# sparisi/pvr_habitat

Measured on AMD Instinct MI355X. Metric: frames/sec embedded (ResNet50, 256x256), higher is better.
Workload: dtype f16; 1 GPU; configs[1]: ResNet50 (MoCo-v2 layout) frozen, 256x256 uint8 frames resident in HBM, batch 256/GPU, random-init synthetic weights, f16 storage / MFMA inputs with fp32 accumulation (the product default, inside the 1e-3 parity bound; configs[1] names bf16); global_batch=256, frame=256, chunk=256, batches_in_flight=2, parallelism=frame shards, no collective (dp1)

## Files before the change

### include/pvr_hip.h

```cpp
#ifndef PVR_HIP_H
#define PVR_HIP_H

#include <stddef.h>
#include <stdint.h>

#ifdef __cplusplus
extern "C" {
#endif

typedef int pvr_status;
#define PVR_OK 0
#define PVR_ERR_INVALID 1
#define PVR_ERR_MISSING_WEIGHT 2
#define PVR_ERR_HIP 3
#define PVR_ERR_STATE 4

#define PVR_BF16 0
#define PVR_F16 1
#define PVR_F32 2
#define PVR_F32S 3

#define PVR_ARCH_RESNET50 0
#define PVR_ARCH_RESNET50_L4 1
#define PVR_ARCH_RESNET50_L3 2
// ... 69 lines not shown
                         const void *residual_dev, void *out_dev, int32_t n, int32_t h, int32_t w,
                         int32_t cin, int32_t cout, int32_t kh, int32_t kw, int32_t stride, int32_t pad,
                         int32_t relu, int32_t out_f32, int32_t dtype, void *hip_stream);
pvr_status pvr_op_conv2d_splitk(const void *in_dev, const void *wgt_dev, const float *bias_dev, const void *residual_dev, void *out_dev, float *scratch_dev,
                                int32_t ksplit, int32_t n, int32_t h, int32_t w, int32_t cin, int32_t cout, int32_t kh, int32_t kw, int32_t stride,
                                int32_t pad, int32_t relu, int32_t out_f32, int32_t dtype, void *hip_stream);
pvr_status pvr_op_bneck_frame(const void *t1_dev, const void *w2_dev, const float *b2_dev, const void *w3_dev, const float *b3_dev,
                              const void *residual_dev, void *y_dev, void *t2_out_dev, const void *w1n_dev, const float *b1n_dev, void *t1n_dev,
                              const void *w1f_dev, const float *b1f_dev, int32_t n, int32_t phases, int32_t dtype, void *hip_stream);
pvr_status pvr_op_pack_frag_weights(const void *w_dev, void *out_dev, int32_t rows, int32_t k, void *hip_stream);
pvr_status pvr_debug_bneck_frame_stamps(const void *t1_dev, const void *w2_dev, const float *b2_dev, const void *w3_dev, const float *b3_dev,
                                        const void *residual_dev, void *y_dev, const void *w1n_dev, const float *b1n_dev, void *t1n_dev,
                                        const void *w1f_dev, const float *b1f_dev, int32_t n, int32_t dtype, uint64_t *stamps_dev, void *hip_stream);
int64_t pvr_debug_bneck_frame_launches(void);
pvr_status pvr_op_conv_wfrag(const void *in_dev, const void *wgt_packed_dev, const float *bias_dev, const void *residual_dev, void *out_dev, int32_t n,
                             int32_t h, int32_t w, int32_t cin, int32_t cout, int32_t kh, int32_t kw, int32_t stride, int32_t pad, int32_t relu,
                             int32_t out_f32, int32_t dtype, void *hip_stream);
pvr_status pvr_op_conv2d_dual(const void *in_dev, const void *in2_dev, const void *wgt_dev, const float *bias_dev, void *out_dev, int32_t n, int32_t h,
                              int32_t w, int32_t cin, int32_t cout, int32_t kh, int32_t kw, int32_t stride, int32_t pad, int32_t h2, int32_t w2,
                              int32_t cin2, int32_t stride2, int32_t relu, int32_t dtype, void *hip_stream);
pvr_status pvr_op_conv_wfrag_pool(const void *in_dev, const void *wgt_packed_dev, const float *bias_dev, const void *residual_dev, float *pool_out_dev,
                                  int64_t pool_stride, int32_t n, int32_t cin, int32_t cout, int32_t dtype, void *hip_stream);
int64_t pvr_debug_conv_wfrag_launches(void);
pvr_status pvr_op_split16_pack_weights(const float *w_dev, void *out_dev, int32_t rows, int32_t k, void *hip_stream);
pvr_status pvr_op_conv2d_split16(const float *in_dev, const void *wgt_split_dev, const float *bias_dev, const float *residual_dev, float *out_dev, int32_t n,
                                 int32_t h, int32_t w, int32_t cin, int32_t cout, int32_t k, int32_t stride, int32_t pad, int32_t relu, void *hip_stream);
pvr_status pvr_op_conv2d_f32(const float *in_dev, const float *wgt_dev, const float *bias_dev, const float *residual_dev, float *out_dev, int32_t n,
                             int32_t h, int32_t w, int32_t cin, int32_t cout, int32_t k, int32_t stride, int32_t pad, int32_t relu, void *hip_stream);
int64_t pvr_debug_conv_split16_launches(void);
pvr_status pvr_op_stem_split16(const float *img_padded_dev, const void *wgt_split_dev, const float *bias_dev, float *out_dev, int32_t n, int32_t S,
                               void *hip_stream);
int64_t pvr_debug_stem_split16_launches(void);
pvr_status pvr_debug_set_conv_algo(int32_t algo);
pvr_status pvr_file_sizes(const char *const *paths, int32_t n, int64_t *sizes, int32_t threads);
pvr_status pvr_read_files(const char *const *paths, int32_t n, uint8_t *dst, const int64_t *offsets, int32_t threads);
pvr_status pvr_stage_copy(void *dst, const void *src, int64_t rows, int64_t row_bytes, int64_t src_row_stride, int64_t run_bytes,
                          int64_t run_stride, int32_t threads);
int64_t pvr_png_scratch_bytes(int32_t n, int32_t h, int32_t w);
pvr_status pvr_png_decode(const uint8_t *files_dev, const int64_t *offsets_dev, int32_t n, int32_t h, int32_t w, uint8_t *out_dev,
                          uint8_t *scratch_dev, int64_t scratch_bytes, int32_t *status_dev, void *hip_stream);

int64_t pvr_debug_conv_expand_launches(void);
int64_t pvr_debug_pp_persistent_launches(void);
pvr_status pvr_op_avgpool(const void *in_dev, float *out_dev, int64_t out_stride, int32_t n, int32_t hw,
                          int32_t c, int32_t in_f32, int32_t dtype, void *hip_stream);
pvr_status pvr_op_avgpool2(const void *in_dev, void *out_dev, int32_t n, int32_t h, int32_t w, int32_t c, int32_t dtype, void *hip_stream);
// ... 21 lines not shown
```

### pvr_habitat_amd/_lib.py

```python
import ctypes as C
import os

_HERE = os.path.dirname(os.path.abspath(__file__))
LIB_PATH = os.environ.get('PVR_LIB') or os.path.join(_HERE, 'lib', 'libpvr_hip.so')

PVR_BF16, PVR_F16, PVR_F32, PVR_F32S = 0, 1, 2, 3
ARCH_RESNET50, ARCH_RESNET50_L4, ARCH_RESNET50_L3 = 0, 1, 2


class EncoderDesc(C.Structure):
    _fields_ = [('arch', C.c_int32), ('dtype', C.c_int32), ('max_batch', C.c_int32), ('chunk', C.c_int32),
                ('resize', C.c_int32), ('crop', C.c_int32), ('mean', C.c_float * 3), ('std_', C.c_float * 3)]


_lib = None

_SIGS = {
    'pvr_version': (C.c_char_p, []),
    'pvr_has_experiments': (C.c_int32, []),
    'pvr_debug_stem_u8_geometry_ok': (C.c_int32, [C.c_void_p, C.c_int32, C.c_int32, C.c_int32, C.c_int32]),
    'pvr_encoder_set_host_backend': (C.c_int, [C.c_void_p, C.c_int32]),
    'pvr_stage_copy': (C.c_int, [C.c_void_p, C.c_void_p, C.c_int64, C.c_int64, C.c_int64, C.c_int64, C.c_int64, C.c_int32]),
    'pvr_last_error': (C.c_size_t, [C.c_char_p, C.c_size_t]),
    'pvr_encoder_create': (C.c_int, [C.POINTER(EncoderDesc), C.POINTER(C.c_void_p)]),
# ... 19 lines not shown
    'pvr_encoder_profile': (C.c_int, [C.c_void_p, C.c_void_p, C.c_int32, C.c_int32, C.c_int32, C.c_void_p, C.c_int64, C.c_void_p,
                                      C.c_void_p, C.c_void_p, C.c_int32, C.POINTER(C.c_int32)]),
    'pvr_encoder_profile_span': (C.c_int, [C.c_void_p, C.c_void_p, C.c_int32, C.c_int32, C.c_int32, C.c_void_p, C.c_int64, C.c_void_p, C.c_int32, C.c_int32,
                                           C.POINTER(C.c_float)]),
    'pvr_op_preprocess': (C.c_int, [C.c_void_p, C.c_int32, C.c_int32, C.c_int32, C.c_int32, C.c_int32, C.c_void_p, C.c_int32, C.c_void_p]),
    'pvr_op_stem': (C.c_int, [C.c_void_p, C.c_void_p, C.c_void_p, C.c_void_p, C.c_int32, C.c_int32, C.c_void_p]),
    'pvr_op_stem_pool': (C.c_int, [C.c_void_p] * 4 + [C.c_int32] * 2 + [C.c_void_p] * 3 + [C.c_int32, C.c_void_p]),
    'pvr_op_stem_pool_u8': (C.c_int, [C.c_void_p] + [C.c_int32] * 5 + [C.c_void_p] * 3 + [C.c_int32] + [C.c_void_p] * 3 + [C.c_int32, C.c_void_p]),
    'pvr_debug_stem_c1_pack': (C.c_int, [C.c_void_p, C.c_void_p]),
    'pvr_op_conv2d_splitk': (C.c_int, [C.c_void_p] * 6 + [C.c_int32] * 13 + [C.c_void_p]),
    'pvr_op_avgpool2': (C.c_int, [C.c_void_p, C.c_void_p] + [C.c_int32] * 5 + [C.c_void_p]),
    'pvr_op_attnpool_tokens': (C.c_int, [C.c_void_p] * 3 + [C.c_int32] * 4 + [C.c_void_p]),
    'pvr_op_nhwc_to_chw': (C.c_int, [C.c_void_p, C.c_void_p, C.c_int64] + [C.c_int32] * 4 + [C.c_void_p]),
    'pvr_op_f32_to_h': (C.c_int, [C.c_void_p, C.c_void_p, C.c_int64, C.c_int32, C.c_void_p]),
    'pvr_op_h_to_f32': (C.c_int, [C.c_void_p, C.c_void_p, C.c_int64, C.c_int32, C.c_void_p]),
    'pvr_op_maxpool': (C.c_int, [C.c_void_p, C.c_void_p, C.c_int32, C.c_int32, C.c_int32, C.c_int32, C.c_int32, C.c_void_p]),
    'pvr_op_conv2d': (C.c_int, [C.c_void_p, C.c_void_p, C.c_void_p, C.c_void_p, C.c_void_p] + [C.c_int32] * 12 + [C.c_void_p]),
    'pvr_op_avgpool': (C.c_int, [C.c_void_p, C.c_void_p, C.c_int64, C.c_int32, C.c_int32, C.c_int32, C.c_int32, C.c_int32, C.c_void_p]),
    'pvr_debug_convert': (C.c_int, [C.c_void_p, C.c_void_p, C.c_int64, C.c_int32]),
    'pvr_op_bneck_frame': (C.c_int, [C.c_void_p] * 13 + [C.c_int32] * 3 + [C.c_void_p]),
    'pvr_debug_bneck_frame_launches': (C.c_int64, []),
    'pvr_op_conv_wfrag': (C.c_int, [C.c_void_p] * 5 + [C.c_int32] * 12 + [C.c_void_p]),
    'pvr_debug_conv_wfrag_launches': (C.c_int64, []),
    'pvr_op_conv_wfrag_pool': (C.c_int, [C.c_void_p] * 5 + [C.c_int64] + [C.c_int32] * 4 + [C.c_void_p]),
    'pvr_op_conv2d_dual': (C.c_int, [C.c_void_p] * 5 + [C.c_int32] * 15 + [C.c_void_p]),
    'pvr_op_pack_frag_weights': (C.c_int, [C.c_void_p, C.c_void_p, C.c_int32, C.c_int32, C.c_void_p]),
    'pvr_debug_bneck_frame_stamps': (C.c_int, [C.c_void_p] * 12 + [C.c_int32] * 2 + [C.c_void_p] * 2),
    'pvr_encoder_check_range': (C.c_int, [C.c_void_p, C.c_void_p, C.c_int32, C.c_int32, C.c_int32, C.c_void_p, C.c_int64, C.c_void_p, C.POINTER(C.c_int32)]),
    'pvr_encoder_debug_set_switch': (C.c_int, [C.c_void_p, C.c_char_p, C.c_int32]),
    'pvr_encoder_launch_kernel': (C.c_int32, [C.c_void_p, C.c_int32, C.c_int32, C.c_char_p, C.c_int32]),
    'pvr_op_split16_pack_weights': (C.c_int, [C.c_void_p, C.c_void_p, C.c_int32, C.c_int32, C.c_void_p]),
    'pvr_op_conv2d_split16': (C.c_int, [C.c_void_p] * 5 + [C.c_int32] * 9 + [C.c_void_p]),
    'pvr_op_conv2d_f32': (C.c_int, [C.c_void_p] * 5 + [C.c_int32] * 9 + [C.c_void_p]),
    'pvr_debug_conv_split16_launches': (C.c_int64, []),
    'pvr_op_stem_split16': (C.c_int, [C.c_void_p] * 4 + [C.c_int32] * 2 + [C.c_void_p]),
    'pvr_debug_stem_split16_launches': (C.c_int64, []),
    'pvr_op_attention': (C.c_int, [C.c_void_p, C.c_void_p, C.c_int32, C.c_int32, C.c_int32, C.c_int32, C.c_int32, C.c_void_p]),
    'pvr_op_layernorm': (C.c_int, [C.c_void_p] * 8 + [C.c_int32] * 3 + [C.c_float, C.c_int32, C.c_int32, C.c_void_p]),
    'pvr_op_cls_head': (C.c_int, [C.c_void_p] * 5 + [C.c_int64] + [C.c_int32] * 4 + [C.c_float, C.c_void_p]),
    'pvr_op_nonfinite_flag': (C.c_int, [C.c_void_p, C.c_int64, C.c_int64, C.c_int64, C.c_void_p, C.c_void_p]),
    'pvr_trainer_create': (C.c_int, [C.POINTER(EncoderDesc), C.POINTER(C.c_void_p)]),
    'pvr_trainer_destroy': (None, [C.c_void_p]),
    'pvr_trainer_out_size': (C.c_int32, [C.c_void_p]),
    'pvr_trainer_param_count': (C.c_int64, [C.c_void_p]),
    'pvr_trainer_workspace_bytes': (C.c_int64, [C.c_void_p]),
    'pvr_trainer_param_name': (C.c_int32, [C.c_void_p, C.c_int32, C.c_char_p, C.c_int32]),
# ... 62 lines not shown
```

### pvr_habitat_amd/csrc/api.hip

```cpp
#include <stdarg.h>
#include "encoder_internal.h"
#include "sample_rng.h"
#include <dlfcn.h>

namespace pvr {

static thread_local std::string g_err;

void set_error(const char *fmt, ...) {
    char buf[1024];
    va_list ap;
    va_start(ap, fmt);
    vsnprintf(buf, sizeof buf, fmt, ap);
    va_end(ap);
    g_err = buf;
}
const std::string &last_error() { return g_err; }

namespace {
typedef int (*roctx_push_fn)(const char *);
typedef int (*roctx_pop_fn)();
struct Roctx {
    roctx_push_fn push = nullptr;
    roctx_pop_fn pop = nullptr;
    Roctx() {
        const char *e = getenv("PVR_ROCTX");
        if (!e || atoi(e) == 0) return;
        for (const char *name : {"librocprofiler-sdk-roctx.so", "librocprofiler-sdk-roctx.so.1", "libroctx64.so", "libroctx64.so.4"}) {
            if (void *h = dlopen(name, RTLD_NOW | RTLD_GLOBAL)) {
                push = (roctx_push_fn)dlsym(h, "roctxRangePushA");
                pop = (roctx_pop_fn)dlsym(h, "roctxRangePop");
                if (push && pop) return;
                push = nullptr; pop = nullptr;
            }
        }
    }
};
const Roctx &roctx() { static Roctx r; return r; }
}
void trace_push(const char *name) { if (roctx().push) roctx().push(name); }
void trace_pop() { if (roctx().pop) roctx().pop(); }

long long conv_expand_launches();
long long bneck_frame_launches();
long long pp_persistent_launches();
long long conv_wfrag_launches();
long long conv_split16_launches();
pvr_status launch_split16_pack(const float *w, void *out, int rows, int K, hipStream_t stream);
pvr_status launch_conv_split16(const float *in, const void *wsp, const float *bias, const float *res, float *out, int n, int h, int w, int cin,
                               int cout, int k, int stride, int pad, int relu, hipStream_t stream, float *out2 = nullptr, int n1 = 0, void *out16 = nullptr,
                               int terms = 3);

static void *g_zero = nullptr;
static pvr_status zero_page(void **out) {
    if (!g_zero) {
        PVR_HIP_TRY(hipMalloc(&g_zero, PVR_ZERO_BYTES));
        PVR_HIP_TRY(hipMemset(g_zero, 0, PVR_ZERO_BYTES));
        PVR_HIP_TRY(hipDeviceSynchronize());
    }
    *out = g_zero;
    return PVR_OK;
}

}

using namespace pvr;

extern "C" {

// ... 18 lines not shown
    return launch_bneck_frame(op_switches(), t1, w2, b2, w3, b3, residual, y, nullptr, n, (w1n ? 7 : 3) | (w1f ? 8 : 0), dtype, (hipStream_t)stream, (unsigned long long *)stamps_dev,
                              w1n, b1n, t1n, w1f, b1f);
}
pvr_status pvr_op_conv_wfrag(const void *in, const void *wgt_packed, const float *bias, const void *residual, void *out, int32_t n, int32_t h, int32_t w,
                             int32_t cin, int32_t cout, int32_t kh, int32_t kw, int32_t stride, int32_t pad, int32_t relu, int32_t out_f32, int32_t dtype,
                             void *stream) {
    PVR_REQUIRE(n > 0 && h > 0 && w > 0, "pvr_op_conv_wfrag: empty input");
    return launch_conv_wfrag(op_switches(), in, wgt_packed, bias, residual, out, n, h, w, cin, cout, kh, kw, stride, pad, relu, out_f32, dtype, (hipStream_t)stream);
}
pvr_status pvr_op_conv2d_dual(const void *in, const void *in2, const void *wgt, const float *bias, void *out, int32_t n, int32_t h, int32_t w, int32_t cin,
                              int32_t cout, int32_t kh, int32_t kw, int32_t stride, int32_t pad, int32_t h2, int32_t w2, int32_t cin2, int32_t stride2,
                              int32_t relu, int32_t dtype, void *stream) {
    PVR_REQUIRE(in && in2 && wgt && bias && out && n > 0, "pvr_op_conv2d_dual: null argument");
    PVR_REQUIRE(dtype == PVR_BF16 || dtype == PVR_F16, "pvr_op_conv2d_dual: 16-bit storage types only");
    return launch_conv_pp256(op_switches(), in, wgt, bias, nullptr, out, n, h, w, cin, cout, kh, kw, stride, pad, relu, 0, 0, dtype, 224, (hipStream_t)stream, in2, h2, w2,
                             cin2, stride2);
}
pvr_status pvr_op_conv_wfrag_pool(const void *in, const void *wgt_packed, const float *bias, const void *residual, float *pool_out, int64_t pool_stride,
                                  int32_t n, int32_t cin, int32_t cout, int32_t dtype, void *stream) {
    PVR_REQUIRE(n > 0 && pool_out, "pvr_op_conv_wfrag_pool: empty input");
    return launch_conv_wfrag(op_switches(), in, wgt_packed, bias, residual, nullptr, n, 7, 7, cin, cout, 1, 1, 1, 0, 1, 1, dtype, (hipStream_t)stream, pool_out, pool_stride);
}
int64_t pvr_debug_conv_wfrag_launches(void) { return (int64_t)conv_wfrag_launches(); }
pvr_status pvr_op_split16_pack_weights(const float *w, void *out, int32_t rows, int32_t k, void *stream) {
    return launch_split16_pack(w, out, rows, k, (hipStream_t)stream);
}
pvr_status pvr_op_conv2d_split16(const float *in, const void *wgt_split, const float *bias, const float *residual, float *out, int32_t n, int32_t h,
                                 int32_t w, int32_t cin, int32_t cout, int32_t k, int32_t stride, int32_t pad, int32_t relu, void *stream) {
    PVR_REQUIRE(n > 0 && h > 0 && w > 0, "pvr_op_conv2d_split16: empty input");
    return launch_conv_split16(in, wgt_split, bias, residual, out, n, h, w, cin, cout, k, stride, pad, relu, (hipStream_t)stream);
}
pvr_status pvr_op_conv2d_f32(const float *in, const float *wgt, const float *bias, const float *residual, float *out, int32_t n, int32_t h, int32_t w,
                             int32_t cin, int32_t cout, int32_t k, int32_t stride, int32_t pad, int32_t relu, void *stream) {
    PVR_REQUIRE(in && wgt && bias && out && n > 0, "pvr_op_conv2d_f32: null argument");
    return launch_conv_f32(in, wgt, bias, residual, out, n, h, w, cin, cout, k, stride, pad, relu, (hipStream_t)stream);
}
int64_t pvr_debug_conv_split16_launches(void) { return (int64_t)conv_split16_launches(); }
pvr_status pvr_op_stem_split16(const float *img_padded, const void *wgt_split, const float *bias, float *out, int32_t n, int32_t S, void *stream) {
    return launch_stem_split16(img_padded, wgt_split, bias, out, n, S, (hipStream_t)stream);
}
int64_t pvr_debug_stem_split16_launches(void) { return (int64_t)stem_split16_launches(); }
int64_t pvr_debug_pp_persistent_launches(void) { return (int64_t)pp_persistent_launches(); }

size_t pvr_last_error(char *buf, size_t cap) {
    const std::string &e = last_error();
    if (buf && cap) {
// ... 168 lines not shown
```

### pvr_habitat_amd/csrc/conv_wfrag.hip

```cpp
#include "encoder_internal.h"

namespace pvr {

struct WFP {
    const u16 *in, *w, *res;
    const float *bias;
    void *out;
    int M, H, W, Cin, Cout, Ho, Wo, KH, KW, stride, pad, act;
    int MT, NCT;
    int nch, cpt;
    int KC;
    int ct_major;
    unsigned in_bytes, w_bytes, out_bytes, res_bytes;
    float *pool_out;
    long long pool_stride;
    int frames;
};

#define WF_LDS_PTR(off_) ((__attribute__((address_space(3))) void *)(smem + (off_)))

template <bool F16, int RES, bool OUT32, int KO = 0, bool POOL = false>
__global__ __launch_bounds__(512, 1) void conv_wfrag_kernel(WFP p) {
    typedef typename HT<F16>::V8 V8;
    constexpr int BMV = POOL ? 98 : 112;
    constexpr int BM = 112, NT = 7, XB = 16384;
    constexpr int OOB = 0x7ffffff0;
    extern __shared__ __attribute__((aligned(16))) char smem[];

    const int tid = threadIdx.x, lane = tid & 63;
    const int wave = __builtin_amdgcn_readfirstlane(tid >> 6);
    const int fr = lane & 15, fq = lane >> 4, sw = (fr >> 1) & 7;
    const int t = xcd_remap(blockIdx.x, gridDim.x);
    int mt, ct;
    if (p.ct_major) { ct = t / p.MT; mt = t - ct * p.MT; }
    else { mt = t / p.NCT; ct = t - mt * p.NCT; }
    const int m0 = mt * BMV, co0 = ct * 256;

    const auto rs_in = __builtin_amdgcn_make_buffer_rsrc(const_cast<u16 *>(p.in), 0, p.in_bytes, 0x00020000);
    const auto rs_w = __builtin_amdgcn_make_buffer_rsrc(const_cast<u16 *>(p.w), 0, p.w_bytes, 0x00020000);
// ... 183 lines not shown
                t += __builtin_bit_cast(float, __builtin_amdgcn_update_dpp(0, __builtin_bit_cast(int, t), 0x114, 0xf, 0xf, true));
                t += __builtin_bit_cast(float, __builtin_amdgcn_update_dpp(0, __builtin_bit_cast(int, t), 0x118, 0xf, 0xf, true));
                tot[e] = t / 49.f;
            }
            const int frame = 2 * mt + f;
            if (fr == 15 && frame < p.frames) {
                float *o = p.pool_out + (long long)frame * p.pool_stride + c;
                *reinterpret_cast<f32x4 *>(o) = f32x4{tot[0], tot[1], tot[2], tot[3]};
                *reinterpret_cast<f32x4 *>(o + 4) = f32x4{tot[4], tot[5], tot[6], tot[7]};
            }
        }
    }
#undef WF_ITER
#undef WF_STEP
#undef WF_XREAD
#undef WF_LOAD_W1
#undef WF_LOAD_W_
#undef WF_LOAD_W
#undef WF_STAGE
#undef WF_STAGE1
#undef WF_STAGE_NEXT
}

static long long g_conv_wfrag_launches = 0;
long long conv_wfrag_launches() { return g_conv_wfrag_launches; }

bool conv_wfrag_supported(int64_t M, int64_t in_bytes, int cin, int cout, int kh, int kw, int pad, int act, int out_f32) {
    const int64_t K = (int64_t)kh * kw * cin;
    return cin % 64 == 0 && cout % 256 == 0 && kh <= 3 && kh == kw && (pad == kh / 2 || pad == 0) && (act == 0 || act == 1) && !(out_f32 & 2) && M >= 1 &&
           M * cout * ((out_f32 & 1) ? 4 : 2) < 0x7ffffff0ll && in_bytes < 0x7ffffff0ll && (int64_t)cout * K * 2 < 0x7ffffff0ll;
}

bool conv_wfrag_preferred(const PlanSwitches &sw, int64_t M, int cin, int cout, int kh, int kw) {
    const int on = sw.conv_wfrag;
    const int64_t K = (int64_t)kh * kw * cin, nct = cout / 256, t256 = ((M + 255) / 256) * nct, t112 = ((M + 111) / 112) * nct;
    if (on == 2) return K >= 512;
    return on && K >= 1024 && t256 < 160 && t112 >= 192;
}

pvr_status launch_conv_wfrag(const PlanSwitches &sw, const void *in, const void *wp, const float *bias, const void *res, void *out, int n, int h, int w, int cin, int cout,
                             int kh, int kw, int stride, int pad, int act, int out_f32, int dtype, hipStream_t stream, float *pool_out, int64_t pool_stride) {
    PVR_REQUIRE(in && wp && bias && (out || pool_out), "conv_wfrag: null argument");
    PVR_REQUIRE(dtype == PVR_BF16 || dtype == PVR_F16, "conv_wfrag: 16-bit storage types only");
    const int ho = (h + 2 * pad - kh) / stride + 1, wo = (w + 2 * pad - kw) / stride + 1;
    const int64_t M = (int64_t)n * ho * wo;
    PVR_REQUIRE(conv_wfrag_supported(M, (int64_t)n * h * w * cin * 2, cin, cout, kh, kw, pad, act, out_f32), "conv_wfrag: unsupported shape");
    WFP p;
    p.in = (const u16 *)in; p.w = (const u16 *)wp; p.res = (const u16 *)res; p.bias = bias; p.out = out;
    p.M = (int)M; p.H = h; p.W = w; p.Cin = cin; p.Cout = cout; p.Ho = ho; p.Wo = wo; p.KH = kh; p.KW = kw; p.stride = stride; p.pad = pad; p.act = act;
    p.MT = pool_out ? (n + 1) / 2 : (int)((M + 111) / 112); p.NCT = cout / 256;
    p.pool_out = pool_out; p.pool_stride = pool_stride; p.frames = n;
    PVR_REQUIRE(!pool_out || (ho == 7 && wo == 7 && res && act == 1 && pool_stride >= cout && ((size_t)pool_out & 15) == 0 && pool_stride % 4 == 0),
                "conv_wfrag: the pooled form is the 7 x 7 conv3 + identity + ReLU of the trunk's last block");
    p.cpt = cin / 64; p.nch = kh * kw * p.cpt; p.KC = kh * kw * cin / 8;
    const int64_t wbytes = (int64_t)cout * kh * kw * cin * 2;
    p.ct_major = wbytes > (5 << 19) ? 1 : 0;
    p.in_bytes = (unsigned)((int64_t)n * h * w * cin * 2); p.w_bytes = (unsigned)wbytes;
    p.out_bytes = (unsigned)(M * cout * ((out_f32 & 1) ? 4 : 2)); p.res_bytes = res ? (unsigned)(M * cout * 2) : 0;
    constexpr int lds = 4 * 16384;
    const dim3 grid((unsigned)(p.MT * p.NCT)), block(512);
    ++g_conv_wfrag_launches;
    const bool f16 = dtype == PVR_F16, o32 = out_f32 & 1;
#define WF_GO(F_, R_, O_) hipLaunchKernelGGL((conv_wfrag_kernel<F_, R_, O_>), grid, block, lds, stream, p)
#ifdef PVR_EXPERIMENTS
    if (sw.wfrag_ko && dtype == PVR_F16 && !res && !(out_f32 & 1)) {
#define WF_KO(k_) case k_: hipLaunchKernelGGL((conv_wfrag_kernel<true, 0, false, k_>), grid, block, lds, stream, p); break;
        switch (sw.wfrag_ko) { WF_KO(1) WF_KO(2) WF_KO(3) WF_KO(4) WF_KO(7) WF_KO(8) WF_KO(9) WF_KO(10) WF_KO(11) WF_KO(15) default: break; }
#undef WF_KO
        PVR_LAUNCH_CHECK();
        return PVR_OK;
    }
#endif
    if (pool_out) {
        if (f16) hipLaunchKernelGGL((conv_wfrag_kernel<true, 1, false, 0, true>), grid, block, lds, stream, p);
        else hipLaunchKernelGGL((conv_wfrag_kernel<false, 1, false, 0, true>), grid, block, lds, stream, p);
        PVR_LAUNCH_CHECK();
        return PVR_OK;
    }
    if (f16) {
        if (res) { if (o32) WF_GO(true, 1, true); else WF_GO(true, 1, false); }
        else { if (o32) WF_GO(true, 0, true); else WF_GO(true, 0, false); }
    } else {
        if (res) { if (o32) WF_GO(false, 1, true); else WF_GO(false, 1, false); }
        else { if (o32) WF_GO(false, 0, true); else WF_GO(false, 0, false); }
    }
#undef WF_GO
    PVR_LAUNCH_CHECK();
    return PVR_OK;
}

}
```

### pvr_habitat_amd/csrc/encoder.hip

```cpp
#include "encoder_internal.h"

namespace pvr {

pvr_status launch_split16_pack(const float *w, void *out, int rows, int K, hipStream_t stream);
pvr_status launch_conv_split16(const float *in, const void *wsp, const float *bias, const float *res, float *out, int n, int h, int w, int cin,
                               int cout, int k, int stride, int pad, int relu, hipStream_t stream, float *out2 = nullptr, int n1 = 0, void *out16 = nullptr,
                               int terms = 3);

void read_switches(PlanSwitches &sw) {
    auto get = [](const char *name, int def) { const char *v = getenv(name); return v ? atoi(v) : def; };
    sw.pool_fuse = get("PVR_POOL_FUSE", 1);
    sw.stem_u8 = get("PVR_STEM_U8", 1);
    sw.stem_lds = get("PVR_STEM_LDS", 1);
    sw.stem_regpool = get("PVR_STEM_REGPOOL", 1);
    sw.frame_front1 = get("PVR_FRAME_FRONT1", 1);
    sw.frame_next1 = get("PVR_FRAME_NEXT1", 0);
    sw.frame_bneck = get("PVR_FRAME_BNECK", 1);
    sw.bneck_stagger = get("PVR_FRAME_STAGGER", 0);
    sw.dual_ds = get("PVR_DUAL_DS", 1);
    sw.chain_ds = get("PVR_CHAIN_DS", 1);
    sw.chain_blocked = get("PVR_CHAIN_BLOCKED", 1);
    sw.chain_halo = get("PVR_CHAIN_HALO", 1);
    sw.chain_ds_occ = get("PVR_CHAIN_DS_OCC", 3);
    sw.chain_pfk = get("PVR_CHAIN_PFK", 12);
    sw.chain_cfg = get("PVR_CHAIN_CFG", 12);
    sw.chain_wave = get("PVR_CHAIN_WAVE", 1);
    sw.chain_wave_halo = get("PVR_CHAIN_WAVE_HALO", 1);
    sw.chain_wave_128 = get("PVR_CHAIN_WAVE_128", 1);
    sw.strided_y = get("PVR_STRIDED_Y", 1);
    sw.splitk = get("PVR_SPLITK", 1);
    sw.smallk_div = get("PVR_SMALLK_DIV", 4);
    if (sw.smallk_div < 1) sw.smallk_div = 1;
    sw.frame_min_n = get("PVR_FRAME_MIN_N", 128);
    sw.frame_run = get("PVR_FRAME_RUN", 0);
    sw.frame_stagger = get("PVR_FRAME_RUN_STAGGER", 0);
    sw.split16 = get("PVR_SPLIT16", 1);
    sw.stem_conv1 = get("PVR_STEM_CONV1", 1);
    sw.resid32 = get("PVR_RESID32", 1);
    sw.tail_f32 = get("PVR_TAIL_F32", 1);
    sw.fuse = get("PVR_FUSE", 1);
    sw.conv_algo = get("PVR_CONV_ALGO", -1);
    sw.conv_halo = get("PVR_CONV_HALO", 1);
    sw.conv_expand = get("PVR_CONV_EXPAND", 1);
    sw.conv_wfrag = get("PVR_CONV_WFRAG", 1);
    sw.wfrag_ko = get("PVR_WFRAG_KO", 0);
    sw.igemm_nk4 = get("PVR_IGEMM_NK4", 1);
    sw.igemm_bm64 = get("PVR_IGEMM_BM64", 0);
    sw.pp_bm224 = get("PVR_PP_BM224", 1);
    sw.pp_persist = get("PVR_PP_PERSIST", 384);
}

PlanSwitches &op_switches() {
    static PlanSwitches sw = [] { PlanSwitches v; read_switches(v); return v; }();
    return sw;
}

template <bool F32>
__global__ __launch_bounds__(256) void range_flag_kernel(const void *x, size_t n8, int dtype, int *flags, int idx) {
    bool bad = false;
    for (size_t i = (size_t)blockIdx.x * 256 + threadIdx.x; i < n8; i += (size_t)gridDim.x * 256) {
        if constexpr (F32) {
            const u32x4 a = reinterpret_cast<const u32x4 *>(x)[2 * i], b = reinterpret_cast<const u32x4 *>(x)[2 * i + 1];
#pragma unroll
            for (int e = 0; e < 4; ++e) bad |= (a[e] & 0x7f800000u) == 0x7f800000u || (b[e] & 0x7f800000u) == 0x7f800000u;
        } else {
            const u32x4 a = reinterpret_cast<const u32x4 *>(x)[i];
            const unsigned em = dtype == PVR_F16 ? 0x7c00u : 0x7f80u;
#pragma unroll
// ... 651 lines not shown
                                    op.h, op.w, op.cin, op.cout, op.k, op.stride, op.pad, op.relu, st, nullptr, 0, (op.out_f32 & 1) ? nullptr : L.buf[op.out_buf], 1);
            break;
        case LK_SPLITK_SMALL:
            s = member(op, L.buf[op.in_buf], res, L.buf[op.out_buf]);
            break;
        case LK_SPLITK:
            s = launch_conv_splitk(L.buf[op.in_buf], op.d_w, op.d_b, res, L.buf[op.out_buf], enc->d_zero, (float *)L.buf[op.ks_buf],
                                   op.ksplit, nb, op.h, op.w, op.cin, op.cout, op.k, op.k, op.stride, op.pad, op.relu, op.out_f32, dt, st);
            break;
        case LK_EXPAND_BLOCKED:
            s = launch_conv_expand(L.buf[op.in_buf], op.d_w, op.d_b, nullptr, L.buf[op.out_buf], nb, op.h, op.w, op.cin, op.cout, 1, op.relu, dt, st, 1);
            t1_blocked = true;
            break;
        case LK_WFRAG_POOL:
            s = launch_conv_wfrag(enc->sw, L.buf[op.in_buf], op.d_wfb, op.d_b, res, nullptr, nb, op.h, op.w, op.cin, op.cout, 1, 1, 1, 0, 1, 1, dt, st,
                                  out, out_stride);
            pooled = true;
            break;
        case LK_WFRAG:
            s = launch_conv_wfrag(enc->sw, L.buf[op.in_buf], op.d_wfb, op.d_b, res, L.buf[op.out_buf], nb, op.h, op.w, op.cin, op.cout, op.k, op.k,
                                  op.stride, op.pad, op.relu, op.out_f32, dt, st);
            break;
        default:
            s = launch_conv(enc->sw, L.buf[op.in_buf], op.d_w, op.d_b, res, L.buf[op.out_buf], enc->d_zero, nb, op.h, op.w,
                            op.cin, op.cout, op.k, op.k, op.stride, op.pad, op.relu, op.out_f32, dt, st);
        }
        if (s) return s;
        if (fa.bad_flags && kind != LK_WFRAG_POOL) {
            const size_t n8 = (size_t)nb * op.ho() * op.wo() * op.cout / 8;
            const int blocks = (int)((n8 + 255) / 256 < 2048 ? (n8 + 255) / 256 : 2048);
            if ((op.out_f32 & 1) || op.f32op) hipLaunchKernelGGL(range_flag_kernel<true>, dim3(blocks), dim3(256), 0, st, L.buf[op.out_buf], n8, dt, fa.bad_flags, (int)li);
            else hipLaunchKernelGGL(range_flag_kernel<false>, dim3(blocks), dim3(256), 0, st, L.buf[op.out_buf], n8, dt, fa.bad_flags, (int)li);
        }
        if ((s = mark())) return s;
        if (!enc->stop_after.empty() && op.tap == enc->stop_after) { stopped = true; break; }
        if (launch_idx++ == stop_idx) { stopped = true; break; }
    }
    enc->last_pooled = pooled;
    if (stopped) return PVR_OK;
    if (pooled)
        s = PVR_OK;
    else if (pooled_head(enc))
        s = launch_avgpool(L.buf[B_F32], out, out_stride, nb, enc->final_hw, enc->final_c, 1, dt, st);
    else
        s = launch_nhwc_to_chw((const float *)L.buf[B_F32], out, out_stride, nb, enc->final_hw, enc->final_c,
                               enc->final_creal, st);
    if (s) return s;
    return mark();
// ... 276 lines not shown
```

### pvr_habitat_amd/csrc/encoder_internal.h

```cpp
#pragma once
#include <map>
#include <string>
#include <vector>
#include <cmath>
#include "common.h"
#include "chain_params.h"

namespace pvr {

struct PlanSwitches {
    int pool_fuse = 1;
    int stem_u8 = 1;
    int stem_lds = 1;
    int stem_regpool = 1;
    int frame_front1 = 1;
    int frame_next1 = 0;
    int frame_bneck = 1;
    int bneck_stagger = 0;
    int dual_ds = 1;
    int chain_ds = 1;
    int chain_blocked = 1;
    int chain_halo = 1;
    int chain_ds_occ = 3;
    int chain_pfk = 12;
    int chain_cfg = 12;
    int chain_wave = 1;
    int chain_wave_halo = 1;
    int chain_wave_128 = 1;
    int strided_y = 1;
    int splitk = 1;
    int smallk_div = 4;
    int frame_run = 0;
    int frame_stagger = 0;
    int frame_min_n = 128;
    int stem_conv1 = 1;
    int split16 = 1;
    int resid32 = 1;
    int tail_f32 = 1;
    int fuse = 1;
    int conv_algo = -1;
    int conv_halo = 1;
    int conv_expand = 1;
    int conv_wfrag = 1;
    int wfrag_ko = 0;
    int igemm_nk4 = 1;
    int igemm_bm64 = 0;
    int pp_bm224 = 1;
    int pp_persist = 384;
};
void read_switches(PlanSwitches &sw);
PlanSwitches &op_switches();

pvr_status launch_preprocess(const uint8_t *, int, int, int, int, int, void *, int, hipStream_t, int crop_pos = 0);
pvr_status launch_stem(const void *, const void *, const float *, void *, int, int, int, hipStream_t);
pvr_status launch_maxpool(const void *, void *, int, int, int, int, int, hipStream_t);
pvr_status launch_stem_pool(const PlanSwitches &sw, const void *, const void *, const float *, void *, int, int, int, hipStream_t, const void *c1_w = nullptr,
                            const float *c1_b = nullptr, void *c1_t1 = nullptr, int c1_blk = 0);
bool stem_pool_u8_ok(const void *, int, int, int, int);
pvr_status launch_stem_pool_u8(const PlanSwitches &sw, const uint8_t *, int, int, int, int, int, const void *, const float *, void *, int, hipStream_t,
                               const void *c1_w = nullptr, const float *c1_b = nullptr, void *c1_t1 = nullptr, int c1_blk = 0);
bool stem_conv1_capable(const PlanSwitches &sw);
void stem_c1_pack(const u16 *w, u16 *img);
void preprocess_geometry(int h, int w, int resize, int crop, int crop_pos, int *resize_needed, int *top, int *left);
pvr_status launch_avgpool(const void *, float *, int64_t, int, int, int, int, int, hipStream_t);
pvr_status launch_nhwc_to_chw(const float *, float *, int64_t, int, int, int, int, hipStream_t);
pvr_status launch_h_to_f32(const void *, float *, size_t, int, hipStream_t);
pvr_status launch_f32_to_h(const float *, void *, size_t, int, hipStream_t);
// ... 5 lines not shown
bool conv_expand_supported(const PlanSwitches &sw, int64_t M, int h, int w, int cin, int cout, int kh, int kw, int stride, int pad, int relu, int out_f32, bool has_res);
pvr_status launch_conv_expand(const void *in, const void *wgt, const float *bias, const void *res, void *out, int n, int h, int w, int cin,
                              int cout, int stride, int relu, int dtype, hipStream_t stream, int out_blk = 0);

bool pp256_supported(int64_t M, int cin, int cout, int kh, int kw, int64_t in_bytes, int64_t w_bytes, int64_t out_bytes, int64_t res_bytes);
pvr_status launch_conv_pp256(const PlanSwitches &sw, const void *in, const void *wgt, const float *bias, const void *res, void *out, int n, int h, int w, int cin,
                             int cout, int kh, int kw, int stride, int pad, int act, int out_f32, int res_f32, int dtype, int bm, hipStream_t stream,
                             const void *in2 = nullptr, int h2 = 0, int w2 = 0, int cin2 = 0, int stride2 = 1);

bool bneck_frame_supported(const PlanSwitches &sw, int n, int h, int w, int cm, int cout, int stride);
pvr_status launch_pack_frag_weights(const void *w, void *out, int rows, int K, hipStream_t stream);
pvr_status launch_bneck_frame(const PlanSwitches &sw, const void *t1, const void *w2p, const float *b2, const void *w3p, const float *b3, const void *res, void *y,
                              void *t2_out, int n, int phases, int dtype, hipStream_t stream, unsigned long long *stamps = nullptr,
                              const void *w1np = nullptr, const float *b1n = nullptr, void *t1n = nullptr, const void *w1fp = nullptr, const float *b1f = nullptr);
struct BFBlk {
    const unsigned short *w1f, *w2, *w3, *res;
    const float *b1f, *b2, *b3;
    unsigned short *y;
};
pvr_status launch_bneck_frame_run(const BFBlk *blocks, int nblk, int n, int dtype, hipStream_t stream, int stagger);

bool conv_wfrag_supported(int64_t M, int64_t in_bytes, int cin, int cout, int kh, int kw, int pad, int act, int out_f32);
bool conv_wfrag_preferred(const PlanSwitches &sw, int64_t M, int cin, int cout, int kh, int kw);
pvr_status launch_conv_wfrag(const PlanSwitches &sw, const void *in, const void *wp, const float *bias, const void *res, void *out, int n, int h, int w, int cin, int cout,
                             int kh, int kw, int stride, int pad, int act, int out_f32, int dtype, hipStream_t stream, float *pool_out = nullptr,
                             int64_t pool_stride = 0);

struct HostTensor {
    std::vector<int64_t> shape;
    std::vector<float> data;
};

inline bool stores_f32(int dtype) { return dtype == PVR_F32 || dtype == PVR_F32S; }

constexpr int PVR_MAX_LANES = 4;
enum BufId { B_NONE = -1, B_X0 = 0, B_X1, B_T1, B_T2, B_DS, B_F32, B_Y0, B_Y1, B_COUNT, B_STEM = B_COUNT };

enum OpRole : uint8_t {
    R_CONV1, R_CONV2, R_CONV3, R_DOWNSAMPLE,
    R_HEAD_CONV1, R_HEAD_DOWNSAMPLE, R_HEAD_CONV2,
    R_STEM_CONV2, R_STEM_CONV3,
    R_AVGPOOL2,
    R_CAST,
};

inline int conv_out_size(int in, int k, int stride, int pad) { return (in + 2 * pad - k) / stride + 1; }
// ... 194 lines not shown
```

Before: 101,700 frames/s.

## Add LDS-resident input 1x1 conv kernel looping over output-channel tiles

Adds a new 1x1 conv kernel for residual 1x1 convs. It loads a block's whole input row tile (all Cin chunks) into LDS once, then walks several 256-wide output-channel tiles while streaming weights. The goal is to stop reloading the same activations for every output-channel tile and to size the grid to roughly one block per CU. The encoder routes eligible conv3 layers, including the final pooled one, to this path when the shape heuristic prefers it. The cost is large LDS use, one block per CU, and more complex register pipelining.

After: 102,500 frames/s, median of 6. About the same (+0.8%).

```diff
diff --git a/include/pvr_hip.h b/include/pvr_hip.h
--- a/include/pvr_hip.h
+++ b/include/pvr_hip.h
@@ -115,6 +115,7 @@
 pvr_status pvr_op_conv_wfrag_pool(const void *in_dev, const void *wgt_packed_dev, const float *bias_dev, const void *residual_dev, float *pool_out_dev,
                                   int64_t pool_stride, int32_t n, int32_t cin, int32_t cout, int32_t dtype, void *hip_stream);
 int64_t pvr_debug_conv_wfrag_launches(void);
+int64_t pvr_debug_conv_wfrag_resident_launches(void);
 pvr_status pvr_op_split16_pack_weights(const float *w_dev, void *out_dev, int32_t rows, int32_t k, void *hip_stream);
 pvr_status pvr_op_conv2d_split16(const float *in_dev, const void *wgt_split_dev, const float *bias_dev, const float *residual_dev, float *out_dev, int32_t n,
                                  int32_t h, int32_t w, int32_t cin, int32_t cout, int32_t k, int32_t stride, int32_t pad, int32_t relu, void *hip_stream);
diff --git a/pvr_habitat_amd/_lib.py b/pvr_habitat_amd/_lib.py
--- a/pvr_habitat_amd/_lib.py
+++ b/pvr_habitat_amd/_lib.py
@@ -65,6 +65,7 @@
     'pvr_debug_bneck_frame_launches': (C.c_int64, []),
     'pvr_op_conv_wfrag': (C.c_int, [C.c_void_p] * 5 + [C.c_int32] * 12 + [C.c_void_p]),
     'pvr_debug_conv_wfrag_launches': (C.c_int64, []),
+    'pvr_debug_conv_wfrag_resident_launches': (C.c_int64, []),
     'pvr_op_conv_wfrag_pool': (C.c_int, [C.c_void_p] * 5 + [C.c_int64] + [C.c_int32] * 4 + [C.c_void_p]),
     'pvr_op_conv2d_dual': (C.c_int, [C.c_void_p] * 5 + [C.c_int32] * 15 + [C.c_void_p]),
     'pvr_op_pack_frag_weights': (C.c_int, [C.c_void_p, C.c_void_p, C.c_int32, C.c_int32, C.c_void_p]),
diff --git a/pvr_habitat_amd/csrc/api.hip b/pvr_habitat_amd/csrc/api.hip
--- a/pvr_habitat_amd/csrc/api.hip
+++ b/pvr_habitat_amd/csrc/api.hip
@@ -45,6 +45,7 @@
 long long bneck_frame_launches();
 long long pp_persistent_launches();
 long long conv_wfrag_launches();
+long long conv_wfrag_resident_launches();
 long long conv_split16_launches();
 pvr_status launch_split16_pack(const float *w, void *out, int rows, int K, hipStream_t stream);
 pvr_status launch_conv_split16(const float *in, const void *wsp, const float *bias, const float *res, float *out, int n, int h, int w, int cin,
@@ -109,6 +110,7 @@
     return launch_conv_wfrag(op_switches(), in, wgt_packed, bias, residual, nullptr, n, 7, 7, cin, cout, 1, 1, 1, 0, 1, 1, dtype, (hipStream_t)stream, pool_out, pool_stride);
 }
 int64_t pvr_debug_conv_wfrag_launches(void) { return (int64_t)conv_wfrag_launches(); }
+int64_t pvr_debug_conv_wfrag_resident_launches(void) { return (int64_t)conv_wfrag_resident_launches(); }
 pvr_status pvr_op_split16_pack_weights(const float *w, void *out, int32_t rows, int32_t k, void *stream) {
     return launch_split16_pack(w, out, rows, k, (hipStream_t)stream);
 }
diff --git a/pvr_habitat_amd/csrc/conv_wfrag.hip b/pvr_habitat_amd/csrc/conv_wfrag.hip
--- a/pvr_habitat_amd/csrc/conv_wfrag.hip
+++ b/pvr_habitat_amd/csrc/conv_wfrag.hip
@@ -15,6 +15,7 @@
     float *pool_out;
     long long pool_stride;
     int frames;
+    int CS, TPW;
 };
 
 #define WF_LDS_PTR(off_) ((__attribute__((address_space(3))) void *)(smem + (off_)))
@@ -244,8 +245,206 @@
 #undef WF_STAGE_NEXT
 }
 
-static long long g_conv_wfrag_launches = 0;
+template <bool F16, bool OUT32, bool POOL>
+__global__ __launch_bounds__(512, 1) void conv_wfrag_resident_kernel(WFP p) {
+    typedef typename HT<F16>::V8 V8;
+    constexpr int BMV = POOL ? 98 : 112;
+    constexpr int BM = 112, NT = 7, XB = 16384;
+    constexpr int OOB = 0x7ffffff0;
+    extern __shared__ __attribute__((aligned(16))) char smem[];
+
+    const int tid = threadIdx.x, lane = tid & 63;
+    const int wave = __builtin_amdgcn_readfirstlane(tid >> 6);
+    const int fr = lane & 15, fq = lane >> 4, sw = (fr >> 1) & 7;
+    const int t = xcd_remap(blockIdx.x, gridDim.x);
+    const int mt = t / p.CS, cs = t - mt * p.CS;
+    const int m0 = mt * BMV;
+    int co0 = cs * p.TPW * 256;
+
+    const auto rs_in = __builtin_amdgcn_make_buffer_rsrc(const_cast<u16 *>(p.in), 0, p.in_bytes, 0x00020000);
+    const auto rs_w = __builtin_amdgcn_make_buffer_rsrc(const_cast<u16 *>(p.w), 0, p.w_bytes, 0x00020000);
+    const auto rs_r = __builtin_amdgcn_make_buffer_rsrc(const_cast<u16 *>(p.res), 0, p.res_bytes, 0x00020000);
+    const auto rs_b = __builtin_amdgcn_make_buffer_rsrc(const_cast<float *>(p.bias), 0, (unsigned)p.Cout * 4u, 0x00020000);
+    const auto rs_o = __builtin_amdgcn_make_buffer_rsrc(p.out, 0, p.out_bytes, 0x00020000);
+
+#pragma unroll
+    for (int i = 0; i < 2; ++i) {
+        const int g = wave + 8 * i, r = g * 8 + (lane >> 3);
+        const int lch = (lane & 7) ^ ((r >> 1) & 7);
+        const int m = m0 + r;
+        const bool ok = g < BM / 8 && r < BMV && m < p.M;
+        const int off = (m * p.Cin + lch * 8) * 2;
+#pragma unroll 1
+        for (int ch = 0; ch < p.nch; ++ch) {
+            __builtin_amdgcn_raw_ptr_buffer_load_lds(rs_in, WF_LDS_PTR(ch * XB + g * 1024), 16, ok ? off + ch * 128 : OOB, 0, 0, 0);
+            asm volatile("" ::: "memory");
+        }
+    }
+
+    const int wlane = lane * 16;
+    int w_rt = (co0 >> 4) + 2 * wave, w_c = 0, w_left = p.TPW * p.nch - 1;
+    V8 w0[2][2], w1[2][2], w2[2][2], w3[2][2];
+#define WR_LOAD_W1(dst_, i_, ks_)                                                                               \
+    {                                                                                                          \
+        dst_[i_][ks_] = __builtin_bit_cast(V8, __builtin_amdgcn_raw_buffer_load_b128(rs_w, wlane, ((w_rt + (i_)) * p.KC + 4 * (2 * w_c + (ks_))) * 256, 0));   \
+        asm volatile("" ::: "memory");                                                                          \
+    }
+#define WR_ADVANCE { if (w_left > 0) { --w_left; if (++w_c == p.nch) { w_c = 0; w_rt += 16; } } }
+#define WR_LOAD_W(dst_) { WR_LOAD_W1(dst_, 0, 0) WR_LOAD_W1(dst_, 0, 1) WR_LOAD_W1(dst_, 1, 0) WR_LOAD_W1(dst_, 1, 1) WR_ADVANCE }
+    u32x4 rr[NT];
+    f32x4 bl, bh;
+#define WR_LOAD_TILE                                                                                            \
+    {                                                                                                          \
+        const int c_ = co0 + 32 * wave + 8 * fq;                                                                \
+        _Pragma("unroll") for (int j = 0; j < NT; ++j) {                                                        \
+            const int m = m0 + 16 * j + fr;                                                                     \
+            rr[j] = __builtin_bit_cast(u32x4, __builtin_amdgcn_raw_buffer_load_b128(rs_r, (m < p.M && 16 * j + fr < BMV) ? (m * p.Cout + c_) * 2 : OOB, 0, 0));   \
+        }                                                                                                       \
+        bl = __builtin_bit_cast(f32x4, __builtin_amdgcn_raw_buffer_load_b128(rs_b, c_ * 4, 0, 0));              \
+        bh = __builtin_bit_cast(f32x4, __builtin_amdgcn_raw_buffer_load_b128(rs_b, c_ * 4 + 16, 0, 0));         \
+        asm volatile("" ::: "memory");                                                                          \
+    }
+    WR_LOAD_W(w0) WR_LOAD_W(w1) WR_LOAD_W(w2)
+    WR_LOAD_TILE
+
+    f32x4 acc[2][NT];
+#pragma unroll
+    for (int i = 0; i < 2; ++i)
+#pragma unroll
+        for (int j = 0; j < NT; ++j) acc[i][j] = f32x4{0.f, 0.f, 0.f, 0.f};
+
+    const int xc = fr * 128 + ((fq ^ sw) << 4), xc64 = xc ^ 64;
+    int ch = 0, tile = 0;
+    int xa = xc, xa64 = xc64, xn, xn64;
+    V8 xs[NT][2];
+    constexpr int RD = 3;
+#define WR_XREAD(j_, a_, a64_)                                                                                  \
+    {                                                                                                          \
+        asm volatile("ds_read_b128 %0, %1 offset:%2" : "=v"(xs[j_][0]) : "v"(a_), "n"((j_) * 2048));            \
+        asm volatile("ds_read_b128 %0, %1 offset:%2" : "=v"(xs[j_][1]) : "v"(a64_), "n"((j_) * 2048));          \
+    }
+#define WR_STEP(q_, W_)                                                                                         \
+    {                                                                                                          \
+        if ((q_) + RD < NT) WR_XREAD((q_) + RD, xa, xa64) else WR_XREAD((q_) + RD - NT, xn, xn64);              \
+        asm volatile("s_waitcnt lgkmcnt(6)" : "+v"(xs[q_][0]), "+v"(xs[q_][1]));                                \
+        __builtin_amdgcn_sched_barrier(0);                                                                      \
+        acc[0][q_] = mfma16<F16>(W_[0][0], xs[q_][0], acc[0][q_]);                                              \
+        acc[1][q_] = mfma16<F16>(W_[1][0], xs[q_][0], acc[1][q_]);                                              \
+        acc[0][q_] = mfma16<F16>(W_[0][1], xs[q_][1], acc[0][q_]);                                              \
+        acc[1][q_] = mfma16<F16>(W_[1][1], xs[q_][1], acc[1][q_]);                                              \
+    }
+#define WR_ITER(W_, WF_)                                                                                        \
+    {                                                                                                          \
+        const int cn_ = ch + 1 == p.nch ? 0 : ch + 1;                                                           \
+        xa = xc + ch * XB; xa64 = xc64 + ch * XB; xn = xc + cn_ * XB; xn64 = xc64 + cn_ * XB;                   \
+        WR_LOAD_W1(WF_, 0, 0) WR_STEP(0, W_)                                                                    \
+        WR_LOAD_W1(WF_, 0, 1) WR_STEP(1, W_)                                                                    \
+        WR_LOAD_W1(WF_, 1, 0) WR_STEP(2, W_)                                                                    \
+        WR_LOAD_W1(WF_, 1, 1) WR_STEP(3, W_)                                                                    \
+        WR_ADVANCE                                                                                              \
+        WR_STEP(4, W_) WR_STEP(5, W_) WR_STEP(6, W_)                                                            \
+        ch = cn_;                                                                                               \
+    }
+#define WR_TILE_END                                                                                             \
+    if (ch == 0) {                                                                                              \
+        const int c = co0 + 32 * wave + 8 * fq;                                                                 \
+        float ps[2][8];                                                                                         \
+        _Pragma("unroll") for (int f = 0; f < 2; ++f)                                                           \
+            _Pragma("unroll") for (int e = 0; e < 8; ++e) ps[f][e] = 0.f;                                       \
+        _Pragma("unroll") for (int j = 0; j < NT; ++j) {                                                        \
+            const int m = m0 + 16 * j + fr;                                                                     \
+            const f32x4 lo = acc[0][j], hi = acc[1][j];                                                         \
+            float v[8] = {lo[0] + bl[0], lo[1] + bl[1], lo[2] + bl[2], lo[3] + bl[3], hi[0] + bh[0], hi[1] + bh[1], hi[2] + bh[2], hi[3] + bh[3]};   \
+            _Pragma("unroll") for (int e = 0; e < 4; ++e) {                                                     \
+                v[2 * e] += from_h<F16>((u16)(rr[j][e] & 0xffffu));                                             \
+                v[2 * e + 1] += from_h<F16>((u16)(rr[j][e] >> 16));                                             \
+            }                                                                                                   \
+            if (p.act) {                                                                                        \
+                _Pragma("unroll") for (int e = 0; e < 8; ++e) v[e] = fmaxf(v[e], 0.f);                          \
+            }                                                                                                   \
+            if constexpr (POOL) {                                                                               \
+                const int pp = 16 * j + fr;                                                                     \
+                _Pragma("unroll") for (int e = 0; e < 8; ++e) {                                                 \
+                    ps[0][e] += pp < 49 ? v[e] : 0.f;                                                           \
+                    ps[1][e] += (pp >= 49 && pp < 98) ? v[e] : 0.f;                                             \
+                }                                                                                               \
+            } else if constexpr (OUT32) {                                                                       \
+                const int o = m < p.M ? (m * p.Cout + c) * 4 : OOB;                                             \
+                __builtin_amdgcn_raw_buffer_store_b128(__builtin_bit_cast(u32x4, f32x4{v[0], v[1], v[2], v[3]}), rs_o, o, 0, 0);    \
+                __builtin_amdgcn_raw_buffer_store_b128(__builtin_bit_cast(u32x4, f32x4{v[4], v[5], v[6], v[7]}), rs_o, o, 16, 0);   \
+            } else {                                                                                            \
+                u32x4 o;                                                                                        \
+                _Pragma("unroll") for (int e = 0; e < 4; ++e) o[e] = (unsigned)to_h<F16>(v[2 * e]) | ((unsigned)to_h<F16>(v[2 * e + 1]) << 16);   \
+                __builtin_amdgcn_raw_buffer_store_b128(o, rs_o, m < p.M ? (m * p.Cout + c) * 2 : OOB, 0, 0);    \
+            }                                                                                                   \
+            acc[0][j] = f32x4{0.f, 0.f, 0.f, 0.f};                                                              \
+            acc[1][j] = f32x4{0.f, 0.f, 0.f, 0.f};                                                              \
+        }                                                                                                       \
+        if constexpr (POOL) {                                                                                   \
+            _Pragma("unroll") for (int f = 0; f < 2; ++f) {                                                     \
+                float tot[8];                                                                                   \
+                _Pragma("unroll") for (int e = 0; e < 8; ++e) {                                                 \
+                    float s_ = ps[f][e];                                                                        \
+                    if (f == 1) s_ = __builtin_bit_cast(float, __builtin_amdgcn_update_dpp(0, __builtin_bit_cast(int, s_), 0x12f, 0xf, 0xf, false));   \
+                    s_ += __builtin_bit_cast(float, __builtin_amdgcn_update_dpp(0, __builtin_bit_cast(int, s_), 0x111, 0xf, 0xf, true));   \
+                    s_ += __builtin_bit_cast(float, __builtin_amdgcn_update_dpp(0, __builtin_bit_cast(int, s_), 0x112, 0xf, 0xf, true));   \
+                    s_ += __builtin_bit_cast(float, __builtin_amdgcn_update_dpp(0, __builtin_bit_cast(int, s_), 0x114, 0xf, 0xf, true));   \
+                    s_ += __builtin_bit_cast(float, __builtin_amdgcn_update_dpp(0, __builtin_bit_cast(int, s_), 0x118, 0xf, 0xf, true));   \
+                    tot[e] = s_ / 49.f;                                                                         \
+                }                                                                                               \
+                const int frame = 2 * mt + f;                                                                   \
+                if (fr == 15 && frame < p.frames) {                                                             \
+                    float *o = p.pool_out + (long long)frame * p.pool_stride + c;                               \
+                    *reinterpret_cast<f32x4 *>(o) = f32x4{tot[0], tot[1], tot[2], tot[3]};                      \
+                    *reinterpret_cast<f32x4 *>(o + 4) = f32x4{tot[4], tot[5], tot[6], tot[7]};                  \
+                }                                                                                               \
+            }                                                                                                   \
+        }                                                                                                       \
+        if (++tile == p.TPW) break;                                                                             \
+        co0 += 256;                                                                                             \
+        WR_LOAD_TILE                                                                                            \
+    }
+
+    asm volatile("s_waitcnt vmcnt(0)" ::: "memory");
+    __builtin_amdgcn_s_barrier();
+    __builtin_amdgcn_sched_barrier(0);
+    WR_XREAD(0, xa, xa64); WR_XREAD(1, xa, xa64); WR_XREAD(2, xa, xa64);
+#pragma unroll 1
+    for (;;) {
+        WR_ITER(w0, w3) WR_TILE_END
+        WR_ITER(w1, w0) WR_TILE_END
+        WR_ITER(w2, w1) WR_TILE_END
+        WR_ITER(w3, w2) WR_TILE_END
+    }
+    asm volatile("s_waitcnt lgkmcnt(0)" ::: "memory");
+#undef WR_TILE_END
+#undef WR_ITER
+#undef WR_STEP
+#undef WR_XREAD
+#undef WR_LOAD_TILE
+#undef WR_LOAD_W
+#undef WR_ADVANCE
+#undef WR_LOAD_W1
+}
+
+static long long g_conv_wfrag_launches = 0, g_conv_wfrag_resident_launches = 0;
 long long conv_wfrag_launches() { return g_conv_wfrag_launches; }
+long long conv_wfrag_resident_launches() { return g_conv_wfrag_resident_launches; }
+
+static int wfrag_resident_split(int64_t MT, int nct) {
+    int cs = 1;
+    for (int d = 1; d <= nct; ++d)
+        if (nct % d == 0 && MT * d <= 256) cs = d;
+    return cs;
+}
+static bool wfrag_resident_shape(const PlanSwitches &sw, int cin, int cout, int kh, int kw, int stride, int pad) {
+    return sw.wfrag_resident && kh == 1 && kw == 1 && stride == 1 && pad == 0 && cin % 64 == 0 && cin <= 512 && cout % 256 == 0;
+}
+bool conv_wfrag_resident_preferred(const PlanSwitches &sw, int64_t M, int cin, int cout) {
+    if (!wfrag_resident_shape(sw, cin, cout, 1, 1, 1, 0) || M < 1) return false;
+    const int64_t MT = (M + 111) / 112;
+    return MT <= 256 && MT * wfrag_resident_split(MT, cout / 256) >= 192;
+}
 
 bool conv_wfrag_supported(int64_t M, int64_t in_bytes, int cin, int cout, int kh, int kw, int pad, int act, int out_f32) {
     const int64_t K = (int64_t)kh * kw * cin;
@@ -271,7 +470,7 @@
     p.in = (const u16 *)in; p.w = (const u16 *)wp; p.res = (const u16 *)res; p.bias = bias; p.out = out;
     p.M = (int)M; p.H = h; p.W = w; p.Cin = cin; p.Cout = cout; p.Ho = ho; p.Wo = wo; p.KH = kh; p.KW = kw; p.stride = stride; p.pad = pad; p.act = act;
     p.MT = pool_out ? (n + 1) / 2 : (int)((M + 111) / 112); p.NCT = cout / 256;
-    p.pool_out = pool_out; p.pool_stride = pool_stride; p.frames = n;
+    p.pool_out = pool_out; p.pool_stride = pool_stride; p.frames = n; p.CS = 1; p.TPW = p.NCT;
     PVR_REQUIRE(!pool_out || (ho == 7 && wo == 7 && res && act == 1 && pool_stride >= cout && ((size_t)pool_out & 15) == 0 && pool_stride % 4 == 0),
                 "conv_wfrag: the pooled form is the 7 x 7 conv3 + identity + ReLU of the trunk's last block");
     p.cpt = cin / 64; p.nch = kh * kw * p.cpt; p.KC = kh * kw * cin / 8;
@@ -293,6 +492,28 @@
         return PVR_OK;
     }
 #endif
+    if (res && !(out_f32 & ~1) && wfrag_resident_shape(sw, cin, cout, kh, kw, stride, pad)) {
+        constexpr int lds_max = 8 * 16384;
+        static DeviceOnce attr_done;
+        if (attr_done.needed()) {
+#define WF_ATTR(F_, O_, P_) PVR_HIP_TRY(hipFuncSetAttribute((const void *)conv_wfrag_resident_kernel<F_, O_, P_>, hipFuncAttributeMaxDynamicSharedMemorySize, lds_max))
+            WF_ATTR(true, false, false); WF_ATTR(true, true, false); WF_ATTR(true, false, true);
+            WF_ATTR(false, false, false); WF_ATTR(false, true, false); WF_ATTR(false, false, true);
+#undef WF_ATTR
+            attr_done.mark();
+        }
+        p.CS = wfrag_resident_split(p.MT, p.NCT); p.TPW = p.NCT / p.CS;
+        const dim3 rgrid((unsigned)(p.MT * p.CS));
+        const int rlds = p.nch * 16384;
+        ++g_conv_wfrag_resident_launches;
+#define WF_RGO(F_, O_, P_) hipLaunchKernelGGL((conv_wfrag_resident_kernel<F_, O_, P_>), rgrid, block, rlds, stream, p)
+        if (pool_out) { if (f16) WF_RGO(true, false, true); else WF_RGO(false, false, true); }
+        else if (o32) { if (f16) WF_RGO(true, true, false); else WF_RGO(false, true, false); }
+        else { if (f16) WF_RGO(true, false, false); else WF_RGO(false, false, false); }
+#undef WF_RGO
+        PVR_LAUNCH_CHECK();
+        return PVR_OK;
+    }
     if (pool_out) {
         if (f16) hipLaunchKernelGGL((conv_wfrag_kernel<true, 1, false, 0, true>), grid, block, lds, stream, p);
         else hipLaunchKernelGGL((conv_wfrag_kernel<false, 1, false, 0, true>), grid, block, lds, stream, p);
diff --git a/pvr_habitat_amd/csrc/encoder.hip b/pvr_habitat_amd/csrc/encoder.hip
--- a/pvr_habitat_amd/csrc/encoder.hip
+++ b/pvr_habitat_amd/csrc/encoder.hip
@@ -44,6 +44,7 @@
     sw.conv_expand = get("PVR_CONV_EXPAND", 1);
     sw.conv_wfrag = get("PVR_CONV_WFRAG", 1);
     sw.wfrag_ko = get("PVR_WFRAG_KO", 0);
+    sw.wfrag_resident = get("PVR_WFRAG_RESIDENT", 1);
     sw.igemm_nk4 = get("PVR_IGEMM_NK4", 1);
     sw.igemm_bm64 = get("PVR_IGEMM_BM64", 0);
     sw.pp_bm224 = get("PVR_PP_BM224", 1);
@@ -741,8 +742,14 @@
                                   op.stride, op.pad, op.relu, op.out_f32, dt, st);
             break;
         default:
-            s = launch_conv(enc->sw, L.buf[op.in_buf], op.d_w, op.d_b, res, L.buf[op.out_buf], enc->d_zero, nb, op.h, op.w,
-                            op.cin, op.cout, op.k, op.k, op.stride, op.pad, op.relu, op.out_f32, dt, st);
+            if (op.wfrag && res && !(op.out_f32 & 2) && op.k == 1 && op.stride == 1 && op.pad == 0 && (dt == PVR_F16 || dt == PVR_BF16) &&
+                conv_wfrag_resident_preferred(enc->sw, (int64_t)nb * op.h * op.w, op.cin, op.cout) &&
+                conv_wfrag_supported((int64_t)nb * op.h * op.w, (int64_t)nb * op.h * op.w * op.cin * 2, op.cin, op.cout, 1, 1, 0, op.relu, op.out_f32))
+                s = launch_conv_wfrag(enc->sw, L.buf[op.in_buf], op.d_wfb, op.d_b, res, L.buf[op.out_buf], nb, op.h, op.w, op.cin, op.cout, 1, 1, 1, 0,
+                                      op.relu, op.out_f32, dt, st);
+            else
+                s = launch_conv(enc->sw, L.buf[op.in_buf], op.d_w, op.d_b, res, L.buf[op.out_buf], enc->d_zero, nb, op.h, op.w,
+                                op.cin, op.cout, op.k, op.k, op.stride, op.pad, op.relu, op.out_f32, dt, st);
         }
         if (s) return s;
         if (fa.bad_flags && kind != LK_WFRAG_POOL) {
diff --git a/pvr_habitat_amd/csrc/encoder_internal.h b/pvr_habitat_amd/csrc/encoder_internal.h
--- a/pvr_habitat_amd/csrc/encoder_internal.h
+++ b/pvr_habitat_amd/csrc/encoder_internal.h
@@ -43,6 +43,7 @@
     int conv_expand = 1;
     int conv_wfrag = 1;
     int wfrag_ko = 0;
+    int wfrag_resident = 1;
     int igemm_nk4 = 1;
     int igemm_bm64 = 0;
     int pp_bm224 = 1;
@@ -94,6 +95,7 @@
 
 bool conv_wfrag_supported(int64_t M, int64_t in_bytes, int cin, int cout, int kh, int kw, int pad, int act, int out_f32);
 bool conv_wfrag_preferred(const PlanSwitches &sw, int64_t M, int cin, int cout, int kh, int kw);
+bool conv_wfrag_resident_preferred(const PlanSwitches &sw, int64_t M, int cin, int cout);
 pvr_status launch_conv_wfrag(const PlanSwitches &sw, const void *in, const void *wp, const float *bias, const void *res, void *out, int n, int h, int w, int cin, int cout,
                              int kh, int kw, int stride, int pad, int act, int out_f32, int dtype, hipStream_t stream, float *pool_out = nullptr,
                              int64_t pool_stride = 0);
```
